# lucidrains/audiolm-pytorch

Measured on AMD Instinct MI355X. Metric: audio-tokens/sec fwd+bwd, CoarseTransformer d=1024 seq=2048, higher is better.
Workload: dtype bf16; 1 GPU; CoarseTransformer dim=1024 depth=6 heads=8 (MQA) num_coarse_quantizers=3 codebook=1024 semantic=500 residual_streams=4 flash_attn=True; per-GPU B=8, N=2048 (509 semantic + 512x3 coarse ids + eos/start); mask_prob=0.15; global_batch=8, seq_len=2048, parallelism=dp1

## Files before the change

audiolm-pytorch_amd/csrc/attention.hip:

```cpp
#include <type_traits>

#include "common.hpp"
#include "../../include/audiolm_hip.h"

namespace {

constexpr int DH = 64;
constexpr float LOG2E = 1.4426950408889634f;
constexpr float RESCALE_THR = 8.0f;
constexpr unsigned OOB = 0x80000000u;
constexpr int HPB = 4;

typedef __attribute__((address_space(3))) void lds_void;

__device__ __forceinline__ int fsw(int row) { return (((row >> 1) & 1) << 2) | (((row >> 3) & 1) << 1) | ((row >> 2) & 1); }

typedef __attribute__((ext_vector_type(4))) float lds_f4v;
typedef __attribute__((ext_vector_type(4))) int lds_i4v;
__device__ __forceinline__ float4 lds_ld_f4(const float* p) {
    const lds_f4v v = *reinterpret_cast<const lds_f4v*>(p);
    return make_float4(v[0], v[1], v[2], v[3]);
}
__device__ __forceinline__ int4 lds_ld_i4(const int* p) {
    const lds_i4v v = *reinterpret_cast<const lds_i4v*>(p);
// ... 390 lines not shown
                }
            PROBE_T(4);
        }
    };
#pragma unroll 1
    for (int tile = 0; tile < ntiles; ++tile) {
        step(smem + ((tile & 1) ^ 1) * 16384, smem + (tile & 1) * 16384, tile);
        __syncthreads();
        PROBE_T(5);
    }

    if (active)
#pragma unroll
    for (int qb = 0; qb < QB; ++qb) {
        const int qi = q0 + qb * 32 + lr;
        const float lt = l[qb] + __shfl_xor(l[qb], 32, 64);
        const float inv = (lt > 0.f ? 1.f / lt : 0.f) * (DROP ? p.drop_scale : 1.f);
        if (qi < p.N) {
            bf16_t* op = p.o + ((long long)b * p.N + qi) * p.ldo + head * DH;
#pragma unroll
            for (int db = 0; db < 2; ++db)
#pragma unroll
                for (int g = 0; g < 4; ++g) {
                    const int d = db * 32 + 8 * g + 4 * lh;
                    *reinterpret_cast<uint2*>(op + d) = make_uint2(pack_bf2(o[db][qb][4 * g] * inv, o[db][qb][4 * g + 1] * inv),
                                                                   pack_bf2(o[db][qb][4 * g + 2] * inv, o[db][qb][4 * g + 3] * inv));
                }
            if (lh == 0) p.lse[((long long)b * p.H + head) * p.N + qi] = (lt > 0.f) ? (m[qb] / LOG2E + logf(lt)) : -INFINITY;
        }
    }
    PROBE_T(6);
    }
    PROBE_FLUSH(blockIdx.x * 4 + wave);
}

__global__ __launch_bounds__(256) void attn_delta_kernel(const bf16_t* __restrict__ o, long long ldo, const bf16_t* __restrict__ dout,
                                                         long long lddo, const float* __restrict__ lse, float* __restrict__ ndelta,
                                                         float* __restrict__ nlse, float inv_scale, int B, int N, int H) {
    const int lane = threadIdx.x & 63;
    const long long row = (long long)blockIdx.x * 4 + (threadIdx.x >> 6);
    if (row >= (long long)B * N) return;
    const int b = (int)(row / N), qi = (int)(row % N);
    for (int c = lane; c < H * 8; c += 64) {
        const bf16x8 a = *reinterpret_cast<const bf16x8*>(o + row * ldo + c * 8);
        const bf16x8 d = *reinterpret_cast<const bf16x8*>(dout + row * lddo + c * 8);
        float s = 0.f;
#pragma unroll
        for (int j = 0; j < 8; ++j) s += bf2f((bf16_t)a[j]) * bf2f((bf16_t)d[j]);
        s += __shfl_xor(s, 1, 64);
        s += __shfl_xor(s, 2, 64);
        s += __shfl_xor(s, 4, 64);
        if ((lane & 7) == 0) {
            const long long idx = ((long long)b * H + (c >> 3)) * N + qi;
            ndelta[idx] = -s;
            const float l = lse[idx];
            nlse[idx] = (l == -INFINITY) ? -INFINITY : -l * inv_scale;
        }
    }
}

template <bool BIAS, bool DROP = false>
__global__ __launch_bounds__(256, 2) void mqa_bwd_dq_kernel(AttnParams p) {
    extern __shared__ __attribute__((aligned(1024))) unsigned char smem[];
    float* kbias = reinterpret_cast<float*>(smem + 32768);
    int* kk4s = reinterpret_cast<int*>(smem + 32768 + 512);
    int* kas = kk4s + 128;
// ... 631 lines not shown
            s0 += pp[(long long)qb * HPB * LT];
            s1 += pp[(long long)(qb + 1) * HPB * LT];
        }
        if (qb < nqb) s0 += pp[(long long)qb * HPB * LT];
    }
    dtbl[(long long)h * LT + t] = (s0 + s1) * scale;
}

}

static int check_attn(int B, int N, int H, long long ldq, long long ldk, long long ldv, long long ldo) {
    if (B <= 0 || N <= 0 || H <= 0 || H > 64) return ALM_ERR_UNSUPPORTED;
    if ((ldq & 7) || (ldk & 7) || (ldv & 7) || (ldo & 3)) return ALM_ERR_BAD_ARG;
    if ((long long)N * ldq * 2 >= 0x7fffffffLL || (long long)N * ldk * 2 >= 0x7fffffffLL || (long long)N * ldv * 2 >= 0x7fffffffLL) return ALM_ERR_UNSUPPORTED;
    const long long ldmax = ldq > ldk ? (ldq > ldv ? ldq : ldv) : (ldk > ldv ? ldk : ldv);
    if ((long long)(N + 64) * (ldmax > ldo ? ldmax : ldo) * 2 >= 0xffffffffLL) return ALM_ERR_UNSUPPORTED;
    return 0;
}

extern "C" int alm_mqa_head_groups(int H) { return (H + HPB - 1) / HPB; }

static int dkv_heads_per_block(int B, int N, int H) {
    static const int env_nh = [] { const char* e = getenv("ALM_ATTN_DKV_NH"); return e ? atoi(e) : 0; }();
    if (env_nh == 2 || env_nh == 4) return env_nh;
    (void)B; (void)H;
    return N >= 8192 ? 2 : HPB;
}
static int dkv_split(int B, int N, int H, int nh) {
    static const int env_sp = [] { const char* e = getenv("ALM_ATTN_DKV_SPLIT"); return e ? atoi(e) : 0; }();
    if (env_sp == 1 || env_sp == 2) return env_sp;
    const long long wgs = (long long)((N + 63) / 64) * ((H + nh - 1) / nh) * B;
    return (N > 64 && 2 * wgs <= 256) ? 2 : 1;
}
extern "C" int alm_mqa_bwd_parts(int B, int N, int H) {
    const int nh = dkv_heads_per_block(B, N, H);
    return ((H + nh - 1) / nh) * dkv_split(B, N, H, nh);
}

struct BiasArgs { const float* tbl; int LT; const int* qkey4; const int* kkey4; const int* qattr; const int* kattr; float* dtbl_part; };

static int check_bias(const BiasArgs& ba, bool bwd) {
    if (!ba.tbl) return 0;
    if (ba.LT < 2 || ba.LT > (1 << 28) || !ba.qkey4 || !ba.kkey4 || !ba.qattr || !ba.kattr || (bwd && !ba.dtbl_part)) return ALM_ERR_BAD_ARG;
    if (((uintptr_t)ba.qkey4 & 15) || ((uintptr_t)ba.qattr & 15)) return ALM_ERR_BAD_ARG;
    return 0;
}

static bool set_dropout(AttnParams& p, float dropout_p, unsigned long long seed, const void* seed_dev) {
    p.seed_dev = nullptr;
    if (!(dropout_p > 0.f)) return false;
    p.seed_dev = reinterpret_cast<const unsigned long long*>(seed_dev);
    const double thr = (double)dropout_p * 4294967296.0;
    p.drop_thr = thr >= 4294967295.0 ? 4294967295u : (unsigned)thr;
    p.drop_scale = 1.f / (1.f - dropout_p);
    p.seed_lo = (unsigned)(seed & 0xffffffffu);
    p.seed_hi = (unsigned)(seed >> 32);
    return true;
}

static int attn_fwd_impl(const void* q, long long ldq, const void* k, long long ldk, const void* v, long long ldv,
                         const unsigned char* mask, void* o, long long ldo, float* lse, int B, int N, int H, int dim_head,
                         float scale, const BiasArgs& ba, float dropout_p, unsigned long long seed, const void* seed_dev, void* stream) {
    if (dropout_p < 0.f || dropout_p >= 1.f) return ALM_ERR_BAD_ARG;
    if (dim_head != DH) return ALM_ERR_UNSUPPORTED;
    int rc = check_attn(B, N, H, ldq, ldk, ldv, ldo);
    if (rc) return rc;
    if (((uintptr_t)q & 15) || ((uintptr_t)k & 15) || ((uintptr_t)v & 15) || ((uintptr_t)o & 7)) return ALM_ERR_BAD_ARG;
    AttnParams p{};
    p.q = (const bf16_t*)q; p.k = (const bf16_t*)k; p.v = (const bf16_t*)v; p.mask = mask; p.o = (bf16_t*)o; p.lse = lse;
    p.ldq = ldq; p.ldk = ldk; p.ldv = ldv; p.ldo = ldo; p.B = B; p.N = N; p.H = H; p.HG = alm_mqa_head_groups(H); p.scale = scale;
    rc = check_bias(ba, false);
    if (rc) return rc;
    p.tbl = ba.tbl; p.LT = ba.LT; p.qkey4 = ba.qkey4; p.kkey4 = ba.kkey4; p.qattr = ba.qattr; p.kattr = ba.kattr;
    const int npair = ((N + 31) / 32 + 1) / 2;
    const bool drop = set_dropout(p, dropout_p, seed, seed_dev);
    static const int qb2_minn = [] { const char* e = getenv("ALM_ATTN_FWD_QB2_MINN"); return e ? atoi(e) : 0; }();
    if (qb2_minn > 0 && N >= qb2_minn && !drop && !p.tbl) {
        hipLaunchKernelGGL((mqa_fwd_kernel<false, 2>), dim3(((N + 63) / 64) * p.HG * B), dim3(256), FWD_LDS<false>, (hipStream_t)stream, p);
        ALM_LAUNCH_CHECK();
        return 0;
    }
    if (drop) {
        if (p.tbl) hipLaunchKernelGGL((mqa_fwd_kernel<true, 1, true>), dim3(npair * p.HG * B), dim3(256), FWD_LDS<true>, (hipStream_t)stream, p);
        else hipLaunchKernelGGL((mqa_fwd_kernel<false, 1, true>), dim3(npair * p.HG * B), dim3(256), FWD_LDS<false>, (hipStream_t)stream, p);
    } else if (p.tbl) hipLaunchKernelGGL((mqa_fwd_kernel<true, 1>), dim3(npair * p.HG * B), dim3(256), FWD_LDS<true>, (hipStream_t)stream, p);
    else hipLaunchKernelGGL((mqa_fwd_kernel<false, 1>), dim3(npair * p.HG * B), dim3(256), FWD_LDS<false>, (hipStream_t)stream, p);
    ALM_LAUNCH_CHECK();
    return 0;
}

static int attn_bwd_impl(const void* q, long long ldq, const void* k, long long ldk, const void* v, long long ldv,
                         const unsigned char* mask, const void* o, long long ldo, const float* lse, const void* dout, long long lddo,
                         void* dq, long long lddq, float* dk, float* dv, long long lddk, long long part_stride, float* delta, int B,
                         int N, int H, int dim_head, float scale, const BiasArgs& ba, float dropout_p, unsigned long long seed, const void* seed_dev, void* stream) {
    if (dim_head != DH) return ALM_ERR_UNSUPPORTED;
    if (dropout_p < 0.f || dropout_p >= 1.f) return ALM_ERR_BAD_ARG;
    int rc = check_attn(B, N, H, ldq, ldk, ldv, ldo);
    if (rc) return rc;
    if ((lddo & 7) || (lddq & 3) || (long long)N * lddo * 2 >= 0x7fffffffLL) return ALM_ERR_BAD_ARG;
    if ((long long)(N + 64) * lddo * 2 >= 0xffffffffLL) return ALM_ERR_UNSUPPORTED;
    rc = check_bias(ba, true);
    if (rc) return rc;
    if (((uintptr_t)q & 15) || ((uintptr_t)k & 15) || ((uintptr_t)v & 15) || ((uintptr_t)dout & 15) || ((uintptr_t)dq & 7)) return ALM_ERR_BAD_ARG;
    hipStream_t st = (hipStream_t)stream;
    float* ndelta = delta;
    float* nlse = delta + (long long)B * H * N;
    hipLaunchKernelGGL(attn_delta_kernel, dim3(((long long)B * N + 3) / 4), dim3(256), 0, st, (const bf16_t*)o, ldo, (const bf16_t*)dout, lddo, lse,
                       ndelta, nlse, 1.0f / scale, B, N, H);
    AttnParams p{};
    p.q = (const bf16_t*)q; p.k = (const bf16_t*)k; p.v = (const bf16_t*)v; p.mask = mask; p.lse = const_cast<float*>(lse);
    p.dout = (const bf16_t*)dout; p.ndelta = ndelta; p.nlse = nlse; p.dq = (bf16_t*)dq; p.dk = dk; p.dv = dv;
// ... 91 lines not shown
```

audiolm-pytorch_amd/csrc/gemm.hip:

```cpp
#include <algorithm>
#include <cstdlib>
#include <type_traits>

#include "common.hpp"
#include "../../include/audiolm_hip.h"

#ifndef ALM_GEMM_AUX_A
#define ALM_GEMM_AUX_A 0
#endif
#ifndef ALM_GEMM_AUX_B
#define ALM_GEMM_AUX_B 0
#endif

namespace {

constexpr int BK = 64;
constexpr unsigned OOB = 0x80000000u;

typedef __attribute__((address_space(3))) void lds_void;

struct GemmParams {
    const bf16_t* A;
    const bf16_t* B;
    void* C;
// ... 650 lines not shown
        }
    }

    const long long coff0 = z1 * p.sC1 + z2 * p.sC2 + (p.ksplit > 0 ? zs * p.sCk : 0);
    GPROBE_T(5);
    gemm_epilogue<BM, BN, WM, WN, TM, TNB, OUT_F32>(p, acc, smem, coff0, m0, n0, wave, wr, wc, lane, lr, lh);
    GPROBE_T(6);
    GPROBE_FLUSH((bx + gridDim.x * (by + gridDim.y * bz)) * 8 + wave);
}


template <bool TNMODE, bool OUT_F32>
__global__ __launch_bounds__(512) void gemm_stag_kernel(GemmParams p) {
    gemm_stag_body<TNMODE, OUT_F32>(p, blockIdx.x, blockIdx.y, blockIdx.z);
}

template <bool OUT_F32>
__global__ __launch_bounds__(512) void gemm_stag_inl_kernel(GemmParams p) {
    gemm_stag_body<false, OUT_F32, true>(p, blockIdx.x, blockIdx.y, blockIdx.z);
}

template <bool TNMODE, bool OUT_F32>
__global__ __launch_bounds__(512) void gemm_stag_group2_kernel(GemmParams p0, GemmParams p1, int tiles0) {
    const bool second = (int)blockIdx.x >= tiles0;
    const GemmParams& p = second ? p1 : p0;
    gemm_stag_body<TNMODE, OUT_F32>(p, second ? (int)blockIdx.x - tiles0 : (int)blockIdx.x, 0, 0);
}

template <bool TNMODE, bool OUT_F32>
__global__ __launch_bounds__(256) void gemm_w4_kernel(GemmParams p) {
    extern __shared__ __attribute__((aligned(1024))) unsigned char smem[];
    GPROBE_DECL
    constexpr int BM = 256, BN = 256, WM = 2, WN = 2, NW = 4, TM = 4, TNB = 4;
    constexpr int A_BYTES = BM * BK * 2, B_BYTES = BN * BK * 2, STAGE = A_BYTES + B_BYTES;
    constexpr int NIA = BM / 8 / NW, NIB = BN / 8 / NW;
    static_assert(NIA + NIB == 16, "the counted waits below assume 16 pieces per wave and stage");

    const int tiles_m = (p.M + BM - 1) / BM, tiles_n = (p.N + BN - 1) / BN;
    int tm, tn, zb, zs;
    if (p.raster >= 1) {
        const int L = blockIdx.x, xcd = L & 7, j = L >> 3;
        const bool m_major = tiles_m >= tiles_n;
        const int tmaj = m_major ? tiles_m : tiles_n, Q = m_major ? tiles_n : tiles_m;
        const int P = p.plimit > 0 ? p.plimit : tmaj * (p.nbt > 0 ? p.nbt : p.nb2);
        const int PL = (P + 7) / 8;
        zs = j / (PL * Q);
        const int rem = j % (PL * Q);
        const int panel = p.raster == 2 ? xcd * PL + rem / Q : (rem / Q) * 8 + xcd;
        const int minor = rem % Q;
        if (panel >= P || zs >= p.nsl) return;
        zb = panel / tmaj;
        const int tmajor = panel % tmaj;
        tm = m_major ? tmajor : minor;
        tn = m_major ? minor : tmajor;
    } else {
        const int nwg = tiles_m * tiles_n;
        const int bid = xcd_remap(blockIdx.x, nwg);
        const int tt = grouped_tile(bid, tiles_m, tiles_n, p.group_m);
        tm = tt & 0xffff;
        tn = tt >> 16;
        zb = blockIdx.y;
        zs = blockIdx.z;
    }
    const int m0 = tm * BM, n0 = tn * BN;
    const int z1 = zb / p.nb2, z2 = zb % p.nb2;
    int kbeg = 0, Krem = p.K;
    const long long zoffA = z1 * p.sA1 + z2 * p.sA2, zoffB = z1 * p.sB1 + z2 * p.sB2;
    if (p.ksplit > 0) {
        kbeg = zs * p.ksplit;
// ... 32 lines not shown
            const int c = (lane & 7) ^ ((row >> 1) & 7);
            offA[j] = (unsigned)(row * p.lda * 2 + c * 16);
            kcA[j] = c * 8;
        }
#pragma unroll
        for (int j = 0; j < NIB; ++j) {
            const int row = (j * NW + wave) * 8 + (lane >> 3);
            const int c = (lane & 7) ^ ((row >> 1) & 7);
            offB[j] = (unsigned)(row * p.ldb * 2 + c * 16);
            kcB[j] = c * 8;
        }
    } else {
        const int st = lane >> 3, kin = (lane >> 1) & 3, half = lane & 1;
#pragma unroll
        for (int j = 0; j < NIA; ++j) {
            const int q = j * NW + wave;
            const int kg = q / (BM / 128), part = q % (BM / 128);
            const int k = kg * 4 + kin, i = part * 128 + st * 16 + half * 8;
            offA[j] = (unsigned)(k * p.lda * 2 + i * 2);
            kcA[j] = k;
        }
#pragma unroll
        for (int j = 0; j < NIB; ++j) {
            const int q = j * NW + wave;
            const int kg = q / (BN / 128), part = q % (BN / 128);
            const int k = kg * 4 + kin, i = part * 128 + st * 16 + half * 8;
            offB[j] = (unsigned)(k * p.ldb * 2 + i * 2);
            kcB[j] = k;
        }
    }
    const unsigned kstepA = TNMODE ? (unsigned)(BK * p.lda * 2) : (unsigned)(BK * 2);
    const unsigned kstepB = TNMODE ? (unsigned)(BK * p.ldb * 2) : (unsigned)(BK * 2);

    auto stage_a = [&](int kt, unsigned char* base) {
        const int kleft = Krem - kt * BK;
#pragma unroll
        for (int j = 0; j < NIA; ++j) {
            const unsigned vo = (kcA[j] < kleft) ? offA[j] : OOB;
            __builtin_amdgcn_raw_ptr_buffer_load_lds(rsA, (lds_void*)(base + (j * NW + wave) * 1024), 16, vo, kt * kstepA, 0, ALM_GEMM_AUX_A);
        }
    };
    auto stage_b = [&](int kt, unsigned char* base) {
        const int kleft = Krem - kt * BK;
#pragma unroll
        for (int j = 0; j < NIB; ++j) {
            const unsigned vo = (kcB[j] < kleft) ? offB[j] : OOB;
            __builtin_amdgcn_raw_ptr_buffer_load_lds(rsB, (lds_void*)(base + A_BYTES + (j * NW + wave) * 1024), 16, vo, kt * kstepB, 0, ALM_GEMM_AUX_B);
        }
    };
    auto stage = [&](int kt, unsigned char* base) { stage_a(kt, base); stage_b(kt, base); };

    unsigned fragA[TM], fragB[TNB];
    if (!TNMODE) {
#pragma unroll
        for (int i = 0; i < TM; ++i) fragA[i] = (unsigned)((wr * 128 + i * 32 + lr) * 128);
#pragma unroll
        for (int j = 0; j < TNB; ++j) fragB[j] = (unsigned)(A_BYTES + (wc * 128 + j * 32 + lr) * 128);
    } else {
        const int g = lane >> 4, s = lane & 15;
#pragma unroll
        for (int i = 0; i < TM; ++i) fragA[i] = (unsigned)((((g >> 1) * 2) * (BM / 16) + (wr * 128 + i * 32) / 16 + (g & 1)) * 128 + s * 8);
#pragma unroll
        for (int j = 0; j < TNB; ++j) fragB[j] = (unsigned)(A_BYTES + (((g >> 1) * 2) * (BN / 16) + (wc * 128 + j * 32) / 16 + (g & 1)) * 128 + s * 8);
    }
    const unsigned sw = (unsigned)((lr >> 1) & 7);

    f32x16 acc[TM][TNB];
#pragma unroll
    for (int i = 0; i < TM; ++i)
#pragma unroll
        for (int j = 0; j < TNB; ++j)
#pragma unroll
            for (int r = 0; r < 16; ++r) acc[i][j][r] = 0.f;

    struct Frags { bf16x8 a[TM], b[TNB]; };
    auto load_frags = [&](const unsigned char* sb, int ks, Frags& f) {
        if (!TNMODE) {
            const unsigned co = (((unsigned)(ks * 2 + lh)) ^ sw) << 4;
#pragma unroll
            for (int i = 0; i < TM; ++i) f.a[i] = *reinterpret_cast<const bf16x8*>(sb + fragA[i] + co);
#pragma unroll
            for (int j = 0; j < TNB; ++j) f.b[j] = *reinterpret_cast<const bf16x8*>(sb + fragB[j] + co);
        } else {
#pragma unroll
            for (int i = 0; i < TM; ++i) {
                const unsigned char* ad = sb + fragA[i] + ks * 4 * (BM / 16) * 128;
                f.a[i] = __builtin_shufflevector(lds_tr16(ad), lds_tr16(ad + (BM / 16) * 128), 0, 1, 2, 3, 4, 5, 6, 7);
            }
#pragma unroll
            for (int j = 0; j < TNB; ++j) {
                const unsigned char* bd = sb + fragB[j] + ks * 4 * (BN / 16) * 128;
                f.b[j] = __builtin_shufflevector(lds_tr16(bd), lds_tr16(bd + (BN / 16) * 128), 0, 1, 2, 3, 4, 5, 6, 7);
            }
        }
    };
    auto mfma_all = [&](const Frags& f) {
#pragma unroll
        for (int i = 0; i < TM; ++i)
#pragma unroll
            for (int j = 0; j < TNB; ++j) acc[i][j] = __builtin_amdgcn_mfma_f32_32x32x16_bf16(f.b[j], f.a[i], acc[i][j], 0, 0, 0);
    };
    constexpr int NMF = TM * TNB;
    constexpr int NRD = (TNMODE ? 2 : 1) * (TM + TNB);

    const int nk = (Krem + BK - 1) / BK;
    Frags F0, F1, F2, F3;

    stage(0, smem);
    if (nk > 1) { stage_a(1, smem + STAGE); wait_vmcnt<8>(); } else wait_vmcnt<0>();
    __builtin_amdgcn_s_barrier();
    load_frags(smem, 0, F0);
    GPROBE_T(0);

    auto kstep = [&](unsigned char* __restrict__ cur, unsigned char* __restrict__ nxt, int kt, auto m2c, auto m1c) {
        constexpr bool MORE2 = decltype(m2c)::value, MORE1 = decltype(m1c)::value;
        if (MORE1) stage_b(kt + 1, nxt);
        load_frags(cur, 1, F1);
        mfma_all(F0);
#pragma unroll
        for (int q = 0; q < NMF / 2; ++q) {
            __builtin_amdgcn_sched_group_barrier(0x008, 2, 0);
            if (MORE1) __builtin_amdgcn_sched_group_barrier(0x010, 1, 0);
            __builtin_amdgcn_sched_group_barrier(0x100, (NRD + NMF / 2 - 1) / (NMF / 2), 0);
        }
        __builtin_amdgcn_sched_barrier(0);
        GPROBE_T(1);
        load_frags(cur, 2, F2);
        mfma_all(F1);
        load_frags(cur, 3, F3);
        mfma_all(F2);
#pragma unroll
        for (int g = 0; g < 2; ++g)
#pragma unroll
            for (int q = 0; q < NMF / 2; ++q) {
                __builtin_amdgcn_sched_group_barrier(0x008, 2, 0);
                __builtin_amdgcn_sched_group_barrier(0x100, (NRD + NMF / 2 - 1) / (NMF / 2), 0);
            }
        __builtin_amdgcn_sched_barrier(0);
        GPROBE_T(2);
        if (MORE1) {
            asm volatile("s_waitcnt vmcnt(0) lgkmcnt(0)" ::: "memory");
            __builtin_amdgcn_s_barrier();
            __builtin_amdgcn_sched_barrier(0);
        }
        GPROBE_T(3);
        if (MORE2) stage_a(kt + 2, cur);
        if (MORE1) load_frags(nxt, 0, F0);
        mfma_all(F3);
#pragma unroll
        for (int q = 0; q < NMF / 2; ++q) {
            __builtin_amdgcn_sched_group_barrier(0x008, 2, 0);
            if (MORE2) __builtin_amdgcn_sched_group_barrier(0x010, 1, 0);
            if (MORE1) __builtin_amdgcn_sched_group_barrier(0x100, (NRD + NMF / 2 - 1) / (NMF / 2), 0);
        }
        __builtin_amdgcn_sched_barrier(0);
        GPROBE_T(4);
    };
    using T = std::true_type;
    using F = std::false_type;
    int kt = 0;
#pragma unroll 1
    for (; kt + 2 < nk; ++kt) kstep(smem + (kt & 1) * STAGE, smem + ((kt & 1) ^ 1) * STAGE, kt, T{}, T{});
    if (kt + 1 < nk) { kstep(smem + (kt & 1) * STAGE, smem + ((kt & 1) ^ 1) * STAGE, kt, F{}, T{}); ++kt; }
    kstep(smem + (kt & 1) * STAGE, smem + ((kt & 1) ^ 1) * STAGE, kt, F{}, F{});
    __syncthreads();

    constexpr int ES = OUT_F32 ? 4 : 2;
    static_assert(NW * 32 * (32 * TNB * ES) <= 2 * STAGE, "epilogue slab");
    const long long coff0 = z1 * p.sC1 + z2 * p.sC2 + (p.ksplit > 0 ? zs * p.sCk : 0);
    gemm_epilogue<BM, BN, WM, WN, TM, TNB, OUT_F32>(p, acc, smem, coff0, m0, n0, wave, wr, wc, lane, lr, lh);
    GPROBE_T(6);
    GPROBE_FLUSH((blockIdx.x + gridDim.x * (blockIdx.y + gridDim.y * blockIdx.z)) * 4 + wave);
}

__global__ __launch_bounds__(256) void splitk_reduce_kernel(const float* __restrict__ ws, int splits, long long mn, long long slice_stride, int N,
                                                            float* __restrict__ C, long long ldc, long long sC, int accumulate,
                                                            int nb2 = 0x40000000, long long sC1 = 0) {
    ws += (long long)blockIdx.y * mn;
    C += (long long)(blockIdx.y / nb2) * sC1 + (long long)(blockIdx.y % nb2) * sC;
    const bool vec = (N & 3) == 0 && (ldc & 3) == 0 && ((uintptr_t)C & 15) == 0 && (mn & 3) == 0 && (slice_stride & 3) == 0;
    if (vec) {
        const long long mn4 = mn >> 2;
        for (long long i = (long long)blockIdx.x * 256 + threadIdx.x; i < mn4; i += (long long)gridDim.x * 256) {
            float4 s = make_float4(0.f, 0.f, 0.f, 0.f);
            for (int z = 0; z < splits; ++z) {
                const float4 v = *reinterpret_cast<const float4*>(ws + (long long)z * slice_stride + i * 4);
                s.x += v.x; s.y += v.y; s.z += v.z; s.w += v.w;
            }
            const long long e = i * 4, m = e / N, n = e % N;
            float4* c = reinterpret_cast<float4*>(C + m * ldc + n);
            if (accumulate) { const float4 w = *c; s.x += w.x; s.y += w.y; s.z += w.z; s.w += w.w; }
            *c = s;
        }
        return;
    }
    for (long long i = (long long)blockIdx.x * 256 + threadIdx.x; i < mn; i += (long long)gridDim.x * 256) {
        float s = 0.f;
        for (int z = 0; z < splits; ++z) s += ws[(long long)z * slice_stride + i];
        const long long m = i / N, n = i % N;
        float* c = C + m * ldc + n;
        *c = accumulate ? *c + s : s;
// ... 223 lines not shown
        hipError_t e = hipFuncSetAttribute(reinterpret_cast<const void*>(kfn), hipFuncAttributeMaxDynamicSharedMemorySize, smem);
        if (e != hipSuccess) return (int)e;
        attr_done = true;
    }
    const int tiles_m = (p.M + 255) / 256, tiles_n = (p.N + 255) / 256;
    if (p.raster >= 1) {
        const int tmaj = tiles_m >= tiles_n ? tiles_m : tiles_n, Q = tiles_m >= tiles_n ? tiles_n : tiles_m;
        const int PL = ((p.plimit > 0 ? p.plimit : tmaj * ny) + 7) / 8;
        hipLaunchKernelGGL(kfn, dim3(8 * PL * Q * nz), dim3(512), smem, st, p);
        return 0;
    }
    hipLaunchKernelGGL(kfn, dim3(tiles_m * tiles_n, ny, nz), dim3(512), smem, st, p);
    return 0;
}


template <bool OUT_F32>
int launch_stag_inl(const GemmParams& p, int ny, hipStream_t st) {
    constexpr int smem = 163840;
    static bool attr_done = false;
    auto kfn = gemm_stag_inl_kernel<OUT_F32>;
    if (!attr_done) {
        hipError_t e = hipFuncSetAttribute(reinterpret_cast<const void*>(kfn), hipFuncAttributeMaxDynamicSharedMemorySize, smem);
        if (e != hipSuccess) return (int)e;
        attr_done = true;
    }
    const int tiles_m = (p.M + 255) / 256, tiles_n = (p.N + 255) / 256;
    hipLaunchKernelGGL(kfn, dim3(tiles_m * tiles_n, ny, p.inl_slices), dim3(512), smem, st, p);
    return 0;
}

template <bool TNMODE, bool OUT_F32>
int launch_w4(const GemmParams& p, int ny, int nz, hipStream_t st) {
    constexpr int smem = 131072;
    static bool attr_done = false;
    auto kfn = gemm_w4_kernel<TNMODE, OUT_F32>;
    if (!attr_done) {
        hipError_t e = hipFuncSetAttribute(reinterpret_cast<const void*>(kfn), hipFuncAttributeMaxDynamicSharedMemorySize, smem);
        if (e != hipSuccess) return (int)e;
        attr_done = true;
    }
    const int tiles_m = (p.M + 255) / 256, tiles_n = (p.N + 255) / 256;
    if (p.raster >= 1) {
        const int tmaj = tiles_m >= tiles_n ? tiles_m : tiles_n, Q = tiles_m >= tiles_n ? tiles_n : tiles_m;
        const int PL = ((p.plimit > 0 ? p.plimit : tmaj * ny) + 7) / 8;
        hipLaunchKernelGGL(kfn, dim3(8 * PL * Q * nz), dim3(256), smem, st, p);
        return 0;
    }
    hipLaunchKernelGGL(kfn, dim3(tiles_m * tiles_n, ny, nz), dim3(256), smem, st, p);
    return 0;
}

int pick_tile(int M, int N, int ny, int tile, bool tn) {
    if (tile == 1 || tile == 2 || tile == 11 || tile == 13 || tile == 14 || tile == 15 || tile == 16 || tile == 17) return tile;
    if (tile != 0) return -1;
    if (M < 256 || N < 256) return 1;
    const long long t256 = (long long)((M + 255) / 256) * ((N + 255) / 256) * ny;
    if (t256 < 192) return 1;
    if (!tn) {
        static const double c320 = [] { const char* e = getenv("ALM_GEMM_T320_COST"); return e ? atoi(e) / 100.0 : 1.22; }();
        const long long t384 = (long long)((M + 383) / 384) * ((N + 255) / 256) * ny;
        const long long t320 = (long long)((M + 319) / 320) * ((N + 255) / 256) * ny;
        const double c13 = (double)((t256 + 255) / 256), c11 = (double)((t384 + 255) / 256) * 1.41;
        const double c17 = c320 > 0. ? (double)((t320 + 255) / 256) * c320 : 1e30;
        if (c17 < c13 && c17 < c11) return 17;
        if (c11 < c13) return 11;
    }
// ... 515 lines not shown
```

Measured before the change: 1.405 million audio-tokens/s.

## Add software-pipelined MQA forward kernel with triple-buffered K/V tiles

Adds a new forward attention kernel that triple-buffers K/V tiles in LDS, processes 64-row query blocks in paired causal passes, and overlaps the QK^T MFMAs of the next tile with the softmax and PV MFMAs of the current tile using sched_group_barrier interleaving. It becomes the default for the no-dropout, no-bias path unless an env var disables it. The aim is to hide LDS/global load latency and exp work behind matrix ops. In exchange it uses more LDS (launch_bounds 256,1 with about 49KB), which may lower occupancy, and it adds a large second code path.

```diff
diff --git a/audiolm-pytorch_amd/csrc/attention.hip b/audiolm-pytorch_amd/csrc/attention.hip
--- a/audiolm-pytorch_amd/csrc/attention.hip
+++ b/audiolm-pytorch_amd/csrc/attention.hip
@@ -446,6 +446,245 @@
     PROBE_T(6);
     }
     PROBE_FLUSH(blockIdx.x * 4 + wave);
+}
+
+constexpr int FWDP_LDS = 3 * 16384 + 3 * 256;
+
+__global__ __launch_bounds__(256, 1) void mqa_fwd_pipe_kernel(AttnParams p) {
+    extern __shared__ __attribute__((aligned(1024))) unsigned char smem[];
+    float* kbias = reinterpret_cast<float*>(smem + 3 * 16384);
+
+    const int nqb = (p.N + 63) / 64;
+    const BlockId id = decode_block(blockIdx.x, (nqb + 1) / 2, p.HG, p.B, true, false);
+    const int b = id.b;
+    const int t = threadIdx.x;
+    const int lane = t & 63;
+    const int wave = __builtin_amdgcn_readfirstlane(t >> 6);
+    const int head = id.hg * HPB + wave;
+    const bool active = head < p.H;
+    const int lr = lane & 31, lh = lane >> 5;
+    const float c2 = p.scale * LOG2E;
+
+    const bf16_t* kbase = p.k + (long long)b * p.N * p.ldk;
+    const bf16_t* vbase = p.v + (long long)b * p.N * p.ldv;
+    const auto rsK = __builtin_amdgcn_make_buffer_rsrc(const_cast<bf16_t*>(kbase), 0, (int)(((long long)(p.N - 1) * p.ldk + DH) * 2), 0x00020000);
+    const auto rsV = __builtin_amdgcn_make_buffer_rsrc(const_cast<bf16_t*>(vbase), 0, (int)(((long long)(p.N - 1) * p.ldv + DH) * 2), 0x00020000);
+    const uint8_t* mrow = p.mask ? p.mask + (long long)b * p.N : nullptr;
+
+    struct KeySide { int raw; };
+    auto load_side = [&](int tile) {
+        KeySide ks{1};
+        if (t < 64) {
+            const int key = tile * 64 + t;
+            ks.raw = key < p.N;
+            if (ks.raw && mrow) ks.raw = mrow[key];
+        }
+        return ks;
+    };
+    auto stage = [&](unsigned char* __restrict__ img, int tile, int slot, const KeySide& ks) {
+        dma_tile<2>(rsK, img, wave, 4, lane, tile * 64, (unsigned)(p.ldk * 2), 0);
+        dma_tile<2>(rsV, img + 8192, wave, 4, lane, tile * 64, (unsigned)(p.ldv * 2), 0);
+        if (t < 64) {
+            int raw = ks.raw;
+            asm volatile("" : "+v"(raw));
+            kbias[slot * 64 + t] = raw ? 0.f : -INFINITY;
+        }
+    };
+
+    const int frow = fsw(lr);
+    const TrOff troff = make_troff(lane);
+    const int npass = (nqb - 1 - id.blk != id.blk) ? 2 : 1;
+    for (int pass = 0; pass < npass; ++pass) {
+    const int qblk = pass ? nqb - 1 - id.blk : id.blk;
+    const int q0 = qblk * 64;
+    const int ntiles = qblk + 1;
+    bf16x8 qf[2][4];
+#pragma unroll
+    for (int qb = 0; qb < 2; ++qb) {
+        const int qi = q0 + qb * 32 + lr;
+        const bf16_t* qp = p.q + ((long long)b * p.N + qi) * p.ldq + head * DH;
+#pragma unroll
+        for (int ks = 0; ks < 4; ++ks) qf[qb][ks] = gload8(qp + ks * 16 + lh * 8, active && qi < p.N);
+    }
+    f32x16 o[2][2];
+#pragma unroll
+    for (int i = 0; i < 2; ++i)
+#pragma unroll
+        for (int j = 0; j < 2; ++j)
+#pragma unroll
+            for (int r = 0; r < 16; ++r) o[i][j][r] = 0.f;
+    float m[2] = {-INFINITY, -INFINITY}, l[2] = {0.f, 0.f}, tm[2];
+
+    auto scores = [&](f32x16 (&s)[2][2], const unsigned char* __restrict__ Kt, int slot) {
+#pragma unroll
+        for (int kb = 0; kb < 2; ++kb)
+#pragma unroll
+            for (int g = 0; g < 4; ++g) {
+                const float4 bv = lds_ld_f4(kbias + slot * 64 + kb * 32 + 8 * g + 4 * lh);
+#pragma unroll
+                for (int qb = 0; qb < 2; ++qb) {
+                    s[kb][qb][4 * g] = bv.x; s[kb][qb][4 * g + 1] = bv.y; s[kb][qb][4 * g + 2] = bv.z; s[kb][qb][4 * g + 3] = bv.w;
+                }
+            }
+#pragma unroll
+        for (int ks = 0; ks < 4; ++ks)
+#pragma unroll
+            for (int kb = 0; kb < 2; ++kb) {
+                const bf16x8 kf = nat_frag(Kt, kb * 32 + lr, frow, ks, lh);
+#pragma unroll
+                for (int qb = 0; qb < 2; ++qb) s[kb][qb] = __builtin_amdgcn_mfma_f32_32x32x16_bf16(kf, qf[qb][ks], s[kb][qb], 0, 0, 0);
+            }
+    };
+    auto causal = [&](f32x16 (&s)[2][2], int tile) {
+        const int doff = tile * 64 - q0;
+#pragma unroll
+        for (int kb = 0; kb < 2; ++kb)
+#pragma unroll
+            for (int qb = 0; qb < 2; ++qb)
+#pragma unroll
+                for (int r = 0; r < 16; ++r)
+                    if (doff + kb * 32 + drow(r, lh) > qb * 32 + lr) s[kb][qb][r] = -INFINITY;
+    };
+    auto tile_max = [&](const f32x16 (&s)[2][2]) {
+#pragma unroll
+        for (int qb = 0; qb < 2; ++qb) {
+            float a = -INFINITY;
+#pragma unroll
+            for (int kb = 0; kb < 2; ++kb)
+#pragma unroll
+                for (int r = 0; r < 16; ++r) a = fmaxf(a, s[kb][qb][r]);
+            a = fmaxf(a, __shfl_xor(a, 32, 64));
+            tm[qb] = a * c2;
+        }
+    };
+
+    f32x16 sa[2][2], sb[2][2];
+    KeySide side = load_side(0);
+    stage(smem, 0, 0, side);
+    side = load_side(1);
+    if (ntiles > 1) {
+        stage(smem + 16384, 1, 1, side);
+        side = load_side(2);
+    }
+    __syncthreads();
+    scores(sa, smem, 0);
+    if (ntiles == 1) causal(sa, 0);
+    tile_max(sa);
+
+    auto body = [&](f32x16 (&sc)[2][2], f32x16 (&sn)[2][2], unsigned char* __restrict__ nimg, const unsigned char* __restrict__ Kn,
+                    const unsigned char* __restrict__ Vc, int tile, int nx, int nn, auto more_c, auto diagn_c) {
+        constexpr bool MORE = decltype(more_c)::value, DIAGN = decltype(diagn_c)::value;
+        if (tile + 2 < ntiles) stage(nimg, tile + 2, nn, side);
+        side = load_side(tile + 3);
+#pragma unroll
+        for (int qb = 0; qb < 2; ++qb) {
+            if (__any(tm[qb] > m[qb] + RESCALE_THR)) {
+                const float mn = fmaxf(m[qb], tm[qb]);
+                const float alpha = (mn == -INFINITY) ? 1.f : __builtin_amdgcn_exp2f(m[qb] - mn);
+                m[qb] = mn;
+                l[qb] *= alpha;
+#pragma unroll
+                for (int db = 0; db < 2; ++db)
+#pragma unroll
+                    for (int r = 0; r < 16; ++r) o[db][qb][r] *= alpha;
+            }
+        }
+        const float ms[2] = {(m[0] == -INFINITY) ? 0.f : m[0], (m[1] == -INFINITY) ? 0.f : m[1]};
+        __builtin_amdgcn_sched_barrier(0);
+        if (MORE) scores(sn, Kn, nx);
+        bf16x8 pf[2][2][2];
+#pragma unroll
+        for (int qb = 0; qb < 2; ++qb) {
+            float ps = 0.f;
+#pragma unroll
+            for (int kb = 0; kb < 2; ++kb)
+#pragma unroll
+                for (int r = 0; r < 16; ++r) {
+                    const float pv = __builtin_amdgcn_exp2f(__builtin_fmaf(sc[kb][qb][r], c2, -ms[qb]));
+                    ps += pv;
+                    sc[kb][qb][r] = pv;
+                }
+            l[qb] += ps;
+#pragma unroll
+            for (int kb = 0; kb < 2; ++kb)
+#pragma unroll
+                for (int s = 0; s < 2; ++s) pf[qb][kb][s] = pack8(sc[kb][qb], s);
+        }
+        if (MORE) {
+#pragma unroll
+            for (int i = 0; i < 16; ++i) {
+                __builtin_amdgcn_sched_group_barrier(0x008, 1, 0);
+                __builtin_amdgcn_sched_group_barrier(0x100, 1, 0);
+                __builtin_amdgcn_sched_group_barrier(0x002, 14, 0);
+            }
+        }
+        __builtin_amdgcn_sched_barrier(0);
+#pragma unroll
+        for (int kb = 0; kb < 2; ++kb)
+#pragma unroll
+            for (int s = 0; s < 2; ++s)
+#pragma unroll
+                for (int db = 0; db < 2; ++db) {
+                    const bf16x8 vf = tr_frag(Vc, kb * 32 + s * 16, troff, db);
+#pragma unroll
+                    for (int qb = 0; qb < 2; ++qb) o[db][qb] = __builtin_amdgcn_mfma_f32_32x32x16_bf16(vf, pf[qb][kb][s], o[db][qb], 0, 0, 0);
+                }
+        if (MORE) {
+            if (DIAGN) causal(sn, tile + 1);
+            tile_max(sn);
+#pragma unroll
+            for (int i = 0; i < 16; ++i) {
+                __builtin_amdgcn_sched_group_barrier(0x008, 1, 0);
+                __builtin_amdgcn_sched_group_barrier(0x100, 1, 0);
+                __builtin_amdgcn_sched_group_barrier(0x002, DIAGN ? 12 : 4, 0);
+            }
+        }
+        __builtin_amdgcn_sched_barrier(0);
+    };
+    auto step = [&](f32x16 (&sc)[2][2], f32x16 (&sn)[2][2], int tile, auto more_c, auto diagn_c) {
+        const int cur = tile % 3, nx = cur == 2 ? 0 : cur + 1, nn = nx == 2 ? 0 : nx + 1;
+        body(sc, sn, smem + nn * 16384, smem + nx * 16384, smem + cur * 16384 + 8192, tile, nx, nn, more_c, diagn_c);
+        __syncthreads();
+    };
+    const std::true_type Y{};
+    const std::false_type F{};
+    int tile = 0;
+#pragma unroll 1
+    for (; tile + 3 < ntiles; tile += 2) {
+        step(sa, sb, tile, Y, F);
+        step(sb, sa, tile + 1, Y, F);
+    }
+    if (tile + 3 == ntiles) {
+        step(sa, sb, tile, Y, F);
+        step(sb, sa, tile + 1, Y, Y);
+        step(sa, sb, tile + 2, F, F);
+    } else if (tile + 2 == ntiles) {
+        step(sa, sb, tile, Y, Y);
+        step(sb, sa, tile + 1, F, F);
+    } else {
+        step(sa, sb, tile, F, F);
+    }
+
+    if (active)
+#pragma unroll
+    for (int qb = 0; qb < 2; ++qb) {
+        const int qi = q0 + qb * 32 + lr;
+        const float lt = l[qb] + __shfl_xor(l[qb], 32, 64);
+        const float inv = lt > 0.f ? 1.f / lt : 0.f;
+        if (qi < p.N) {
+            bf16_t* op = p.o + ((long long)b * p.N + qi) * p.ldo + head * DH;
+#pragma unroll
+            for (int db = 0; db < 2; ++db)
+#pragma unroll
+                for (int g = 0; g < 4; ++g) {
+                    const int d = db * 32 + 8 * g + 4 * lh;
+                    *reinterpret_cast<uint2*>(op + d) = make_uint2(pack_bf2(o[db][qb][4 * g] * inv, o[db][qb][4 * g + 1] * inv),
+                                                                   pack_bf2(o[db][qb][4 * g + 2] * inv, o[db][qb][4 * g + 3] * inv));
+                }
+            if (lh == 0) p.lse[((long long)b * p.H + head) * p.N + qi] = (lt > 0.f) ? (m[qb] / LOG2E + logf(lt)) : -INFINITY;
+        }
+    }
+    }
 }
 
 __global__ __launch_bounds__(256) void attn_delta_kernel(const bf16_t* __restrict__ o, long long ldo, const bf16_t* __restrict__ dout,
@@ -1143,6 +1382,12 @@
     const long long wgs = (long long)((N + 63) / 64) * ((H + nh - 1) / nh) * B;
     return (N > 64 && 2 * wgs <= 256) ? 2 : 1;
 }
+static bool attn_fwd_pipe(int B, int N, int H) {
+    static const int env_pipe = [] { const char* e = getenv("ALM_ATTN_FWD_PIPE"); return e ? atoi(e) : -1; }();
+    if (env_pipe == 0 || env_pipe == 1) return env_pipe == 1;
+    (void)B; (void)N; (void)H;
+    return true;
+}
 extern "C" int alm_mqa_bwd_parts(int B, int N, int H) {
     const int nh = dkv_heads_per_block(B, N, H);
     return ((H + nh - 1) / nh) * dkv_split(B, N, H, nh);
@@ -1188,6 +1433,12 @@
     static const int qb2_minn = [] { const char* e = getenv("ALM_ATTN_FWD_QB2_MINN"); return e ? atoi(e) : 0; }();
     if (qb2_minn > 0 && N >= qb2_minn && !drop && !p.tbl) {
         hipLaunchKernelGGL((mqa_fwd_kernel<false, 2>), dim3(((N + 63) / 64) * p.HG * B), dim3(256), FWD_LDS<false>, (hipStream_t)stream, p);
+        ALM_LAUNCH_CHECK();
+        return 0;
+    }
+    if (!drop && !p.tbl && attn_fwd_pipe(B, N, H)) {
+        const int npair64 = ((N + 63) / 64 + 1) / 2;
+        hipLaunchKernelGGL(mqa_fwd_pipe_kernel, dim3(npair64 * p.HG * B), dim3(256), FWDP_LDS, (hipStream_t)stream, p);
         ALM_LAUNCH_CHECK();
         return 0;
     }
```

Result: slower. 1.379 million audio-tokens/s, median of 2 (-1.8%).

## Triple-buffer B tiles and interleave LDS loads with MFMA groups in w4 GEMM

Applied to the files above, without the earlier changes.

Reworks the 256x256 four-wave GEMM main loop. A stays double-buffered while B gets three LDS buffers, so B for step k+2 is prefetched two iterations ahead. The coarse sched_group_barrier hints are replaced by explicit interleaving: every pair of MFMAs is followed by individual fragment reads or buffer-load pieces, fenced with sched_barrier. LDS use grows from 128 KiB to 160 KiB per block, which can limit occupancy and adds more complex counted waits.

```diff
diff --git a/audiolm-pytorch_amd/csrc/gemm.hip b/audiolm-pytorch_amd/csrc/gemm.hip
--- a/audiolm-pytorch_amd/csrc/gemm.hip
+++ b/audiolm-pytorch_amd/csrc/gemm.hip
@@ -706,9 +706,9 @@
     extern __shared__ __attribute__((aligned(1024))) unsigned char smem[];
     GPROBE_DECL
     constexpr int BM = 256, BN = 256, WM = 2, WN = 2, NW = 4, TM = 4, TNB = 4;
-    constexpr int A_BYTES = BM * BK * 2, B_BYTES = BN * BK * 2, STAGE = A_BYTES + B_BYTES;
+    constexpr int A_BYTES = BM * BK * 2, B_BYTES = BN * BK * 2;
     constexpr int NIA = BM / 8 / NW, NIB = BN / 8 / NW;
-    static_assert(NIA + NIB == 16, "the counted waits below assume 16 pieces per wave and stage");
+    static_assert(NIA == 8 && NIB == 8 && 2 * A_BYTES + 3 * B_BYTES == 163840, "the counted waits below assume 8 + 8 pieces; LDS map");
 
     const int tiles_m = (p.M + BM - 1) / BM, tiles_n = (p.N + BN - 1) / BN;
     int tm, tn, zb, zs;
@@ -807,36 +807,18 @@
     const unsigned kstepA = TNMODE ? (unsigned)(BK * p.lda * 2) : (unsigned)(BK * 2);
     const unsigned kstepB = TNMODE ? (unsigned)(BK * p.ldb * 2) : (unsigned)(BK * 2);
 
-    auto stage_a = [&](int kt, unsigned char* base) {
-        const int kleft = Krem - kt * BK;
-#pragma unroll
-        for (int j = 0; j < NIA; ++j) {
-            const unsigned vo = (kcA[j] < kleft) ? offA[j] : OOB;
-            __builtin_amdgcn_raw_ptr_buffer_load_lds(rsA, (lds_void*)(base + (j * NW + wave) * 1024), 16, vo, kt * kstepA, 0, ALM_GEMM_AUX_A);
-        }
-    };
-    auto stage_b = [&](int kt, unsigned char* base) {
-        const int kleft = Krem - kt * BK;
-#pragma unroll
-        for (int j = 0; j < NIB; ++j) {
-            const unsigned vo = (kcB[j] < kleft) ? offB[j] : OOB;
-            __builtin_amdgcn_raw_ptr_buffer_load_lds(rsB, (lds_void*)(base + A_BYTES + (j * NW + wave) * 1024), 16, vo, kt * kstepB, 0, ALM_GEMM_AUX_B);
-        }
-    };
-    auto stage = [&](int kt, unsigned char* base) { stage_a(kt, base); stage_b(kt, base); };
-
     unsigned fragA[TM], fragB[TNB];
     if (!TNMODE) {
 #pragma unroll
         for (int i = 0; i < TM; ++i) fragA[i] = (unsigned)((wr * 128 + i * 32 + lr) * 128);
 #pragma unroll
-        for (int j = 0; j < TNB; ++j) fragB[j] = (unsigned)(A_BYTES + (wc * 128 + j * 32 + lr) * 128);
+        for (int j = 0; j < TNB; ++j) fragB[j] = (unsigned)((wc * 128 + j * 32 + lr) * 128);
     } else {
         const int g = lane >> 4, s = lane & 15;
 #pragma unroll
         for (int i = 0; i < TM; ++i) fragA[i] = (unsigned)((((g >> 1) * 2) * (BM / 16) + (wr * 128 + i * 32) / 16 + (g & 1)) * 128 + s * 8);
 #pragma unroll
-        for (int j = 0; j < TNB; ++j) fragB[j] = (unsigned)(A_BYTES + (((g >> 1) * 2) * (BN / 16) + (wc * 128 + j * 32) / 16 + (g & 1)) * 128 + s * 8);
+        for (int j = 0; j < TNB; ++j) fragB[j] = (unsigned)((((g >> 1) * 2) * (BN / 16) + (wc * 128 + j * 32) / 16 + (g & 1)) * 128 + s * 8);
     }
     const unsigned sw = (unsigned)((lr >> 1) & 7);
 
@@ -849,99 +831,113 @@
             for (int r = 0; r < 16; ++r) acc[i][j][r] = 0.f;
 
     struct Frags { bf16x8 a[TM], b[TNB]; };
-    auto load_frags = [&](const unsigned char* sb, int ks, Frags& f) {
+    auto read_frag = [&](const unsigned char* sa, const unsigned char* sbb, int ks, int f, Frags& fr) {
+        const bool is_a = f == 0 || f >= 5;
+        const int x = f == 0 ? 0 : (f >= 5 ? f - 4 : f - 1);
         if (!TNMODE) {
             const unsigned co = (((unsigned)(ks * 2 + lh)) ^ sw) << 4;
-#pragma unroll
-            for (int i = 0; i < TM; ++i) f.a[i] = *reinterpret_cast<const bf16x8*>(sb + fragA[i] + co);
-#pragma unroll
-            for (int j = 0; j < TNB; ++j) f.b[j] = *reinterpret_cast<const bf16x8*>(sb + fragB[j] + co);
+            if (is_a) fr.a[x] = *reinterpret_cast<const bf16x8*>(sa + fragA[x] + co);
+            else fr.b[x] = *reinterpret_cast<const bf16x8*>(sbb + fragB[x] + co);
+        } else if (is_a) {
+            const unsigned char* ad = sa + fragA[x] + ks * 4 * (BM / 16) * 128;
+            fr.a[x] = __builtin_shufflevector(lds_tr16(ad), lds_tr16(ad + (BM / 16) * 128), 0, 1, 2, 3, 4, 5, 6, 7);
         } else {
-#pragma unroll
-            for (int i = 0; i < TM; ++i) {
-                const unsigned char* ad = sb + fragA[i] + ks * 4 * (BM / 16) * 128;
-                f.a[i] = __builtin_shufflevector(lds_tr16(ad), lds_tr16(ad + (BM / 16) * 128), 0, 1, 2, 3, 4, 5, 6, 7);
-            }
-#pragma unroll
-            for (int j = 0; j < TNB; ++j) {
-                const unsigned char* bd = sb + fragB[j] + ks * 4 * (BN / 16) * 128;
-                f.b[j] = __builtin_shufflevector(lds_tr16(bd), lds_tr16(bd + (BN / 16) * 128), 0, 1, 2, 3, 4, 5, 6, 7);
-            }
+            const unsigned char* bd = sbb + fragB[x] + ks * 4 * (BN / 16) * 128;
+            fr.b[x] = __builtin_shufflevector(lds_tr16(bd), lds_tr16(bd + (BN / 16) * 128), 0, 1, 2, 3, 4, 5, 6, 7);
         }
     };
-    auto mfma_all = [&](const Frags& f) {
-#pragma unroll
-        for (int i = 0; i < TM; ++i)
-#pragma unroll
-            for (int j = 0; j < TNB; ++j) acc[i][j] = __builtin_amdgcn_mfma_f32_32x32x16_bf16(f.b[j], f.a[i], acc[i][j], 0, 0, 0);
+    auto substep = [&](const Frags& fc, auto&& extra) {
+#pragma unroll
+        for (int g = 0; g < 8; ++g) {
+            const int i = g / 2, j0 = (g % 2) * 2;
+            acc[i][j0] = __builtin_amdgcn_mfma_f32_32x32x16_bf16(fc.b[j0], fc.a[i], acc[i][j0], 0, 0, 0);
+            acc[i][j0 + 1] = __builtin_amdgcn_mfma_f32_32x32x16_bf16(fc.b[j0 + 1], fc.a[i], acc[i][j0 + 1], 0, 0, 0);
+            __builtin_amdgcn_sched_barrier(0);
+            extra(g);
+            __builtin_amdgcn_sched_barrier(0);
+        }
     };
-    constexpr int NMF = TM * TNB;
-    constexpr int NRD = (TNMODE ? 2 : 1) * (TM + TNB);
-
+    auto piece_a = [&](int kt, unsigned char* buf, int j) {
+        const unsigned vo = (kcA[j] < Krem - kt * BK) ? offA[j] : OOB;
+        __builtin_amdgcn_raw_ptr_buffer_load_lds(rsA, (lds_void*)(buf + (j * NW + wave) * 1024), 16, vo, kt * kstepA, 0, ALM_GEMM_AUX_A);
+    };
+    auto piece_b = [&](int kt, unsigned char* buf, int j) {
+        const unsigned vo = (kcB[j] < Krem - kt * BK) ? offB[j] : OOB;
+        __builtin_amdgcn_raw_ptr_buffer_load_lds(rsB, (lds_void*)(buf + (j * NW + wave) * 1024), 16, vo, kt * kstepB, 0, ALM_GEMM_AUX_B);
+    };
+
+    unsigned char* const abuf0 = smem;
+    unsigned char* const bbuf0 = smem + 2 * A_BYTES;
     const int nk = (Krem + BK - 1) / BK;
     Frags F0, F1, F2, F3;
 
-    stage(0, smem);
-    if (nk > 1) { stage_a(1, smem + STAGE); wait_vmcnt<8>(); } else wait_vmcnt<0>();
+#pragma unroll
+    for (int j = 0; j < NIA; ++j) piece_a(0, abuf0, j);
+#pragma unroll
+    for (int j = 0; j < NIB; ++j) piece_b(0, bbuf0, j);
+    if (nk > 1) {
+#pragma unroll
+        for (int j = 0; j < NIB; ++j) piece_b(1, bbuf0 + B_BYTES, j);
+#pragma unroll
+        for (int j = 0; j < NIA; ++j) piece_a(1, abuf0 + A_BYTES, j);
+        wait_vmcnt<16>();
+    } else {
+        wait_vmcnt<0>();
+    }
     __builtin_amdgcn_s_barrier();
-    load_frags(smem, 0, F0);
+    __builtin_amdgcn_sched_barrier(0);
+#pragma unroll
+    for (int f = 0; f < 8; ++f) read_frag(abuf0, bbuf0, 0, f, F0);
     GPROBE_T(0);
 
-    auto kstep = [&](unsigned char* __restrict__ cur, unsigned char* __restrict__ nxt, int kt, auto m2c, auto m1c) {
+    auto kstep = [&](unsigned char* __restrict__ a_cur, unsigned char* __restrict__ a_nxt, unsigned char* __restrict__ b_cur,
+                     unsigned char* __restrict__ b_nxt, unsigned char* __restrict__ b_far, int kt, auto m2c, auto m1c) {
         constexpr bool MORE2 = decltype(m2c)::value, MORE1 = decltype(m1c)::value;
-        if (MORE1) stage_b(kt + 1, nxt);
-        load_frags(cur, 1, F1);
-        mfma_all(F0);
-#pragma unroll
-        for (int q = 0; q < NMF / 2; ++q) {
-            __builtin_amdgcn_sched_group_barrier(0x008, 2, 0);
-            if (MORE1) __builtin_amdgcn_sched_group_barrier(0x010, 1, 0);
-            __builtin_amdgcn_sched_group_barrier(0x100, (NRD + NMF / 2 - 1) / (NMF / 2), 0);
-        }
-        __builtin_amdgcn_sched_barrier(0);
+        substep(F0, [&](int g) {
+            if (g < 4) { read_frag(a_cur, b_cur, 1, 2 * g, F1); read_frag(a_cur, b_cur, 1, 2 * g + 1, F1); }
+            if (MORE2 && (g & 1) == 0) piece_b(kt + 2, b_far, g / 2);
+        });
         GPROBE_T(1);
-        load_frags(cur, 2, F2);
-        mfma_all(F1);
-        load_frags(cur, 3, F3);
-        mfma_all(F2);
-#pragma unroll
-        for (int g = 0; g < 2; ++g)
-#pragma unroll
-            for (int q = 0; q < NMF / 2; ++q) {
-                __builtin_amdgcn_sched_group_barrier(0x008, 2, 0);
-                __builtin_amdgcn_sched_group_barrier(0x100, (NRD + NMF / 2 - 1) / (NMF / 2), 0);
-            }
-        __builtin_amdgcn_sched_barrier(0);
+        substep(F1, [&](int g) {
+            if (g < 4) { read_frag(a_cur, b_cur, 2, 2 * g, F2); read_frag(a_cur, b_cur, 2, 2 * g + 1, F2); }
+            if (MORE2 && (g & 1) == 0) piece_b(kt + 2, b_far, 4 + g / 2);
+        });
+        substep(F2, [&](int g) {
+            if (g < 4) { read_frag(a_cur, b_cur, 3, 2 * g, F3); read_frag(a_cur, b_cur, 3, 2 * g + 1, F3); }
+        });
         GPROBE_T(2);
         if (MORE1) {
-            asm volatile("s_waitcnt vmcnt(0) lgkmcnt(0)" ::: "memory");
+            if (MORE2) wait_vmcnt<8>(); else wait_vmcnt<0>();
+            asm volatile("s_waitcnt lgkmcnt(0)" ::: "memory");
             __builtin_amdgcn_s_barrier();
             __builtin_amdgcn_sched_barrier(0);
         }
         GPROBE_T(3);
-        if (MORE2) stage_a(kt + 2, cur);
-        if (MORE1) load_frags(nxt, 0, F0);
-        mfma_all(F3);
-#pragma unroll
-        for (int q = 0; q < NMF / 2; ++q) {
-            __builtin_amdgcn_sched_group_barrier(0x008, 2, 0);
-            if (MORE2) __builtin_amdgcn_sched_group_barrier(0x010, 1, 0);
-            if (MORE1) __builtin_amdgcn_sched_group_barrier(0x100, (NRD + NMF / 2 - 1) / (NMF / 2), 0);
-        }
-        __builtin_amdgcn_sched_barrier(0);
+        substep(F3, [&](int g) {
+            if (MORE2) piece_a(kt + 2, a_cur, g);
+            if (MORE1 && g < 4) { read_frag(a_nxt, b_nxt, 0, 2 * g, F0); read_frag(a_nxt, b_nxt, 0, 2 * g + 1, F0); }
+        });
         GPROBE_T(4);
     };
     using T = std::true_type;
     using F = std::false_type;
-    int kt = 0;
+    int kt = 0, bc = 0;
+    auto bb = [&](int q) { return bbuf0 + (q >= 3 ? q - 3 : q) * B_BYTES; };
 #pragma unroll 1
-    for (; kt + 2 < nk; ++kt) kstep(smem + (kt & 1) * STAGE, smem + ((kt & 1) ^ 1) * STAGE, kt, T{}, T{});
-    if (kt + 1 < nk) { kstep(smem + (kt & 1) * STAGE, smem + ((kt & 1) ^ 1) * STAGE, kt, F{}, T{}); ++kt; }
-    kstep(smem + (kt & 1) * STAGE, smem + ((kt & 1) ^ 1) * STAGE, kt, F{}, F{});
+    for (; kt + 2 < nk; ++kt) {
+        kstep(abuf0 + (kt & 1) * A_BYTES, abuf0 + ((kt & 1) ^ 1) * A_BYTES, bb(bc), bb(bc + 1), bb(bc + 2), kt, T{}, T{});
+        bc = bc == 2 ? 0 : bc + 1;
+    }
+    if (kt + 1 < nk) {
+        kstep(abuf0 + (kt & 1) * A_BYTES, abuf0 + ((kt & 1) ^ 1) * A_BYTES, bb(bc), bb(bc + 1), bb(bc + 2), kt, F{}, T{});
+        ++kt;
+        bc = bc == 2 ? 0 : bc + 1;
+    }
+    kstep(abuf0 + (kt & 1) * A_BYTES, abuf0 + ((kt & 1) ^ 1) * A_BYTES, bb(bc), bb(bc + 1), bb(bc + 2), kt, F{}, F{});
     __syncthreads();
 
     constexpr int ES = OUT_F32 ? 4 : 2;
-    static_assert(NW * 32 * (32 * TNB * ES) <= 2 * STAGE, "epilogue slab");
+    static_assert(NW * 32 * (32 * TNB * ES) <= 2 * A_BYTES + 3 * B_BYTES, "epilogue slab");
     const long long coff0 = z1 * p.sC1 + z2 * p.sC2 + (p.ksplit > 0 ? zs * p.sCk : 0);
     gemm_epilogue<BM, BN, WM, WN, TM, TNB, OUT_F32>(p, acc, smem, coff0, m0, n0, wave, wr, wc, lane, lr, lh);
     GPROBE_T(6);
@@ -1231,7 +1227,7 @@
 
 template <bool TNMODE, bool OUT_F32>
 int launch_w4(const GemmParams& p, int ny, int nz, hipStream_t st) {
-    constexpr int smem = 131072;
+    constexpr int smem = 163840;
     static bool attr_done = false;
     auto kfn = gemm_w4_kernel<TNMODE, OUT_F32>;
     if (!attr_done) {
```

Result: no change. 1.489 million audio-tokens/s before, 1.504 million audio-tokens/s after, median of 6 (+1.0%).
